# mit-acl/clipper

Hardware: AMD Instinct MI355X
Metric: affinity+solve ms and GEMV HBM GB/s, n=10k assoc, 95% outliers, 1/8 GPU (lower is better)
Workload: dtype f64 (M stored f32)

## Files before the change

### clipper_amd/build.py

```python
from __future__ import annotations

import os
import shutil
import subprocess
import sys
import sysconfig

HERE = os.path.dirname(os.path.abspath(__file__))
ROOT = os.path.dirname(HERE)
CSRC = os.path.join(HERE, "csrc")
LIBDIR = os.path.join(HERE, "lib")
HIP_LIB = os.path.join(LIBDIR, "libclipper_hip.so")
WAVE_CHECK_SRC = os.path.join(ROOT, "tests", "hip", "wave_check.hip")
WAVE_CHECK = os.path.join(ROOT, "tools", "_bin", "wave_check")

HIPCC = shutil.which("hipcc") or "/opt/rocm/bin/hipcc"
HIP_FLAGS = ["--offload-arch=gfx950", "-O3", "-std=c++17", "-ffp-contract=off", "-fPIC",
             "-shared", "-Wall", "-Wno-unused-value"]


def _newer(target: str, sources: list[str]) -> bool:
    if not os.path.exists(target):
        return False
    t = os.path.getmtime(target)
    return all(os.path.getmtime(s) <= t for s in sources if os.path.exists(s))


def _run(cmd: list[str]):
    print("+", " ".join(cmd), flush=True)
    subprocess.check_call(cmd)


def hip_sources() -> list[str]:
    return [os.path.join(dp, f) for top in (CSRC, os.path.join(ROOT, "include")) for dp, _, fs in os.walk(top)
            for f in fs if f.endswith((".hip", ".h", ".hpp"))]


def build_hip(force: bool = False) -> str:
    os.makedirs(LIBDIR, exist_ok=True)
    if force or not _newer(HIP_LIB, hip_sources()):
        _run([HIPCC, *HIP_FLAGS, "-o", HIP_LIB, os.path.join(CSRC, "clipper_hip.hip"), "-ldl"])
    return HIP_LIB


def pymodule_path() -> str:
    return os.path.join(LIBDIR, "clipperpy" + (sysconfig.get_config_var("EXT_SUFFIX") or ".so"))


def build_pymodule(force: bool = False) -> str | None:
    host = os.path.join(CSRC, "host")
    src = os.path.join(host, "py_clipper.cpp")
    if not os.path.exists(src):
        return None
    import pybind11
    out = pymodule_path()
    srcs = [src, os.path.join(host, "clipper.cpp"), os.path.join(host, "batch.cpp")] + [
        os.path.join(dp, f) for dp, _, fs in os.walk(os.path.join(ROOT, "include")) for f in fs]
    if force or not _newer(out, srcs + [HIP_LIB]):
        _run(["g++", "-O2", "-std=c++17", "-fPIC", "-shared", "-fvisibility=hidden", "-fopenmp",
              "-DCLIPPER_NO_EIGEN",
              "-I", os.path.join(ROOT, "include"), "-I", pybind11.get_include(),
              "-I", sysconfig.get_paths()["include"],
              src, os.path.join(host, "clipper.cpp"), os.path.join(host, "batch.cpp"),
              "-L", LIBDIR, "-lclipper_hip", "-Wl,-rpath,$ORIGIN", "-o", out])
    return out


def build_wave_check(force: bool = False) -> str:
    os.makedirs(os.path.dirname(WAVE_CHECK), exist_ok=True)
    if force or not _newer(WAVE_CHECK, hip_sources() + [WAVE_CHECK_SRC]):
        _run([HIPCC, *[f for f in HIP_FLAGS if f not in ("-shared", "-fPIC")], "-I", CSRC, "-o", WAVE_CHECK, WAVE_CHECK_SRC])
    return WAVE_CHECK


def build_all(force: bool = False):
    build_hip(force)
    build_pymodule(force)
    build_wave_check(force)


if __name__ == "__main__":
    build_all(force="--force" in sys.argv)
```

### clipper_amd/csrc/host_plan.hpp

```cpp
#pragma once

#include <algorithm>
#include <cmath>
#include <cstdint>
#include <cstdlib>
#include <vector>

namespace clipper_plan {

struct Work {
  int strip, slot, t0, t1;
  int q0, q1, pad0, pad1;
};

struct PassConsts {
  int nw;
  int so;
  int occ = 6;
  int per_strip = 12;
};

struct PassPlan {
  std::vector<Work> work;
  int nslots = 1;
// ... 237 lines not shown
        const size_t wv = ui * NWV + static_cast<size_t>(wave);
        out.wave_cg[wv] = static_cast<uint8_t>(cgl);
        int rem = (sub == nw[cgl] - 1) ? (1 << 30) : target, n = 0;
        while (rem > 0 && kcur < U.k1) {
          const int mq = static_cast<int>(lrow[kcur] & 255u);
          if (qcur >= mq) {
            ++kcur;
            qcur = 0;
            continue;
          }
          if (n == K.pmax) {
            if (sub == nw[cgl] - 1) return;
            break;
          }
          const int take = std::min(rem, mq - qcur);
          out.pieces[wv * PM + static_cast<size_t>(n++)] = static_cast<uint32_t>(kcur - U.k0) |
                                                           (static_cast<uint32_t>(qcur) << 8) |
                                                           (static_cast<uint32_t>(qcur + take) << 16);
          qcur += take;
          rem -= take;
        }
        out.npieces[wv] = static_cast<uint8_t>(n);
      }
    }
  }
  out.ok = true;
}


struct ViewUnit {
  int cg0, ncgs;
  int l0, l1;
  int pack;
  int pad1, pad2, pad3;
};

struct ViewResidentPlan {
  bool ok = false;
  uint32_t lds_slices = 0;
  uint64_t entries = 0;
  std::vector<ViewUnit> units;
  std::vector<uint8_t> npieces;
  std::vector<uint8_t> wave_cg;
  std::vector<uint32_t> pieces;
  std::vector<uint64_t> ent, byt;
  std::vector<int> stp, sorted_stp, T, nw;
};

inline void plan_view_resident(const uint32_t* L, int ncg, int nchunks, int esize, int target_units, int max_units,
                               uint32_t fixed_bytes, const ResidentConsts& K, ViewResidentPlan& out) {
  out.ok = false;
  out.units.clear();
  out.entries = 0;
  if (ncg < 1 || nchunks < 1 || nchunks > K.tmax || fixed_bytes + K.slice_pad + 8192 >= K.lds_max) return;
  const uint32_t cap = K.lds_max - fixed_bytes - K.slice_pad;
  out.lds_slices = K.lds_max - fixed_bytes;
  const uint32_t QBY = 4u * static_cast<uint32_t>(esize);
  std::vector<uint64_t>&ent = out.ent, &byt = out.byt;
  ent.assign(static_cast<size_t>(ncg), 0);
  byt.assign(static_cast<size_t>(ncg), 0);
  uint64_t total = 0;
  for (int cg = 0; cg < ncg; ++cg) {
    uint64_t e = 0, b = 0;
    for (int k = 0; k < nchunks; ++k) {
      const uint32_t lq = L[static_cast<size_t>(cg) * nchunks + k];
      e += lq >> 8;
      b += slice_bound(lq, QBY, K.so);
    }
    ent[static_cast<size_t>(cg)] = e;
    byt[static_cast<size_t>(cg)] = b;
    total += e;
  }
  out.entries = total;
  target_units = std::max(1, std::min(target_units, max_units));
  const double Te0 = std::max(256.0, static_cast<double>(total) / target_units);
  const int max_cgs = std::min(K.nwv, K.tmax / nchunks);
  if (max_cgs < 1) return;
  std::vector<int>&stp = out.stp, &sorted_stp = out.sorted_stp;
  stp.assign(static_cast<size_t>(ncg), 0);
  for (int c = 0; c < ncg; ++c) {
    int t = 0;
    for (int k = 0; k < nchunks; ++k) t += static_cast<int>(L[static_cast<size_t>(c) * nchunks + k] & 255u);
    stp[static_cast<size_t>(c)] = t;
  }
  sorted_stp = stp;
// ... 76 lines not shown
          best = cgl;
      ++nw[static_cast<size_t>(best)];
    }
    int wave = 0;
    for (int cgl = 0; cgl < U.ncgs; ++cgl) {
      const int nwc = nw[static_cast<size_t>(cgl)];
      const int target = std::max(1, (T[static_cast<size_t>(cgl)] + nwc - 1) / nwc);
      int kcur = 0, qcur = 0;
      for (int sub = 0; sub < nwc; ++sub, ++wave) {
        const size_t wv = ui * NWV + static_cast<size_t>(wave);
        out.wave_cg[wv] = static_cast<uint8_t>(cgl);
        int rem = (sub == nwc - 1) ? (1 << 30) : target, n = 0;
        while (rem > 0 && kcur < nsl) {
          const int mq = steps_of(cgl, kcur);
          if (qcur >= mq) {
            ++kcur;
            qcur = 0;
            continue;
          }
          if (n == K.pmax) {
            if (sub == nwc - 1) return;
            break;
          }
          const int take = std::min(rem, mq - qcur);
          out.pieces[wv * PM + static_cast<size_t>(n++)] = static_cast<uint32_t>(kcur) | (static_cast<uint32_t>(qcur) << 8) |
                                                           (static_cast<uint32_t>(qcur + take) << 16);
          qcur += take;
          rem -= take;
        }
        out.npieces[wv] = static_cast<uint8_t>(n);
      }
    }
  }
  out.ok = true;
}

}
```

### clipper_amd/csrc/host_rv_resident.hpp

```cpp
#pragma once

namespace {

void rvr_begin_solve(Ctx* h) {
  ViewResident& r = h->vres;
  r.launches_this_solve = 0;
  r.ev_n = 0;
  if (r.giveup_host) std::memset(r.giveup_host, 0, RVR_GIVEUP_SLOTS * 4 * sizeof(uint32_t));
  std::atomic_thread_fence(std::memory_order_seq_cst);
}

void rvr_end_solve(Ctx* h) {
  ViewResident& r = h->vres;
  if (r.cooldown > 0 && r.launches_this_solve == 0) --r.cooldown;
  if (r.launches_this_solve == 0 || !r.giveup_host) return;
  std::atomic_thread_fence(std::memory_order_acquire);
  int gave_up = 0;
  volatile const uint32_t* w = r.giveup_host;
  for (int k = 0; k < std::min(r.launches_this_solve, RVR_GIVEUP_SLOTS); ++k) {
    if (w[4 * k] != 0u) {
      ++gave_up;
    } else {
      h->rv_stats.resident_iterations += static_cast<int64_t>(w[4 * k + 1]);
      h->rv_stats.resident_us += static_cast<double>(static_cast<uint64_t>(w[4 * k + 2]) | (static_cast<uint64_t>(w[4 * k + 3]) << 32)) * 1e-2;
// ... 21 lines not shown
}

bool rvr_gate(const Ctx* h) { return h->rv_mode == 0 && csc_possible(h) && h->sh.size() == 1 && (h->V == 6 || h->V == 4); }
bool rvr_local_ok(const Ctx* h) {
  static const bool env_off = [] {
    const char* e = std::getenv("CLIPPER_HIP_VIEW_RESIDENT");
    return e && std::atoi(e) == 0;
  }();
  return !env_off && h->vres.cooldown == 0;
}
bool rvr_common(const Ctx* h) { return rvr_gate(h) && rvr_local_ok(h); }
bool rvr_enabled(const Ctx* h) { return rvr_common(h) && csc_single(h); }
bool rvr_replica_gate(const Ctx* h) { return rvr_gate(h) && h->multiproc && rect_fill_possible(h); }
bool rvr_replica_enabled(const Ctx* h) { return rvr_replica_gate(h) && rvr_local_ok(h); }

bool rvr_candidate(const Ctx* h, int64_t nrows) { return rvr_enabled(h) && nrows >= 1 && nrows <= RVR_MAXROWS; }

int rvr_plan(Ctx* h, Shard& s, bool replica = false) {
  ViewResident& r = h->vres;
  r.ready = false;
  r.on_replica = replica;
  if (!(replica ? rvr_replica_enabled(h) && s.rv.full_valid : rvr_enabled(h)) || !s.rv.valid) return 0;
  const RowView& v = s.rv;
  const SliceStore& vst = replica ? v.full : v.st;
  if (v.nrows < 1 || v.nrows > RVR_MAXROWS) return 0;
  static_assert(sizeof(clipper_plan::ViewUnit) == sizeof(RvrUnit), "the planner's unit is the kernel's");
  const clipper_plan::ResidentConsts K{RVR_NT, RVR_NWV, RVR_TMAX, RVR_PMAX, 2, RS_LDS_MAX,
                                       RVR_RED_BYTES, RVR_TAB_BYTES, RS_SLICE_PAD, SL_SO};
  static thread_local clipper_plan::ViewResidentPlan plan;
  if (r.target_units == 0) {
    const char* e = std::getenv("CLIPPER_HIP_VIEW_RESIDENT_WGS");
    r.target_units = e ? std::max(1, std::atoi(e)) : -1;
  }
  if (r.max_units_device < 0) {
    int per_cu = 0;
    hipError_t e = hipErrorUnknown;
    dispatch_vt(h, [&](auto tag) {
      using VT = decltype(tag);
      auto kern = (h->V == 6) ? k_solve_view_resident<VT, 6, false> : k_solve_view_resident<VT, 4, false>;
      if (raise_dynamic_lds(reinterpret_cast<const void*>(kern), s.device, static_cast<int>(RS_LDS_MAX)))
        e = hipOccupancyMaxActiveBlocksPerMultiprocessor(&per_cu, reinterpret_cast<const void*>(kern), RVR_NT, RS_LDS_MAX);
    });
    if (e != hipSuccess) (void)hipGetLastError();
    r.max_units_device = (e == hipSuccess) ? per_cu * h->cus : 0;
    if (rs_debug()) std::fprintf(stderr, "[view-resident] the device holds %d workgroups of the kernel at a time\n", r.max_units_device);
  }
  if (r.max_units_device < 16) return 0;
  const int max_units = std::min({RVR_MAXUNITS, h->cus - 8, r.max_units_device - 8});
  const int target = r.target_units > 0 ? r.target_units : std::max(8, (2 * h->cus) / 3);
  const uint32_t fixed = rvr_xt_bytes(h->V, static_cast<int>(v.nrows)) + RVR_RED_BYTES + RVR_TAB_BYTES;
  clipper_plan::plan_view_resident(h->csc_hLq, vst.s_ncg, vst.s_nchunks, static_cast<int>(h->esize()), target,
                                   max_units, fixed, K, plan);
  if (rs_debug())
    std::fprintf(stderr, "[view-resident] plan rows=%lld ncg=%d nchunks=%d entries=%llu -> units=%zu ok=%d\n",
                 static_cast<long long>(v.nrows), vst.s_ncg, vst.s_nchunks,
                 static_cast<unsigned long long>(plan.entries), plan.units.size(), plan.ok ? 1 : 0);
  if (!plan.ok) return 0;
  if (rs_debug() && std::atoi(std::getenv("CLIPPER_HIP_RESIDENT_DEBUG")) >= 2) {
    for (size_t ui = 0; ui < plan.units.size(); ++ui) {
      const clipper_plan::ViewUnit& U = plan.units[ui];
      uint64_t ent = 0;
      for (int c = 0; c < U.ncgs; ++c) ent += plan.ent[static_cast<size_t>(U.cg0 + c)];
      if (U.l1 - U.l0 < 64) ent = ent * static_cast<uint64_t>(U.l1 - U.l0) / 64;
      int wmax = 0, wsum = 0;
      for (int w = 0; w < RVR_NWV; ++w) {
        int st = 0;
        for (int j = 0; j < plan.npieces[ui * RVR_NWV + w]; ++j) {
          const uint32_t pc = plan.pieces[(ui * RVR_NWV + w) * RVR_PMAX + j];
          st += static_cast<int>((pc >> 16) & 255u) - static_cast<int>((pc >> 8) & 255u);
        }
        wmax = std::max(wmax, st);
        wsum += st;
      }
      std::fprintf(stderr, "[view-resident-unit] %zu cg0 %d ncgs %d lanes %d-%d pack %d entries %llu steps_max_wave %d steps_sum %d\n", ui, U.cg0, U.ncgs,
                   U.l0, U.l1, U.pack, static_cast<unsigned long long>(ent), wmax, wsum);
    }
  }
  HIPCHK(hipSetDevice(s.device));
  const size_t off_np = plan.units.size() * sizeof(RvrUnit);
  const size_t off_wc = off_np + static_cast<size_t>(round_up(static_cast<int64_t>(plan.npieces.size()), 16));
  const size_t off_pc = off_wc + static_cast<size_t>(round_up(static_cast<int64_t>(plan.wave_cg.size()), 16));
  const size_t bytes = off_pc + plan.pieces.size() * sizeof(uint32_t) + 64;
  if (bytes > r.host_plan.cap) HIPCHK(r.host_plan.alloc(bytes + 4096, hipHostMallocMapped | hipHostMallocCoherent));
  std::memcpy(r.host_plan, plan.units.data(), plan.units.size() * sizeof(RvrUnit));
  std::memcpy(r.host_plan + off_np, plan.npieces.data(), plan.npieces.size());
  std::memcpy(r.host_plan + off_wc, plan.wave_cg.data(), plan.wave_cg.size());
  {
    uint32_t* dst = reinterpret_cast<uint32_t*>(r.host_plan + off_pc);
    const uint32_t* src = plan.pieces.data();
    for (size_t wv = 0; wv < plan.npieces.size(); ++wv)
      for (int j = 0; j < plan.npieces[wv]; ++j) dst[wv * RVR_PMAX + j] = src[wv * RVR_PMAX + j];
  }
  std::atomic_thread_fence(std::memory_order_seq_cst);
  r.off_np = off_np;
  r.off_wc = off_wc;
  r.off_pc = off_pc;
  const size_t xb_bytes = static_cast<size_t>(rvr_xb_granules(6)) * sizeof(unsigned long long);
  if (!r.xb) {
    HIPCHK(r.xb.alloc(xb_bytes / sizeof(unsigned long long)));
    HIPCHK(hipMemsetAsync(r.xb, 0, xb_bytes, s.stream));
  }
  if (!r.ctl) {
    HIPCHK(r.ctl.alloc(RVR_GIVEUP_SLOTS * 16));
    HIPCHK(hipMemsetAsync(r.ctl, 0, RVR_GIVEUP_SLOTS * 64, s.stream));
  }
  if (!r.giveup_host) {
    HIPCHK(r.giveup_host.alloc(RVR_GIVEUP_SLOTS * 4, hipHostMallocMapped | hipHostMallocCoherent));
    std::memset(r.giveup_host, 0, RVR_GIVEUP_SLOTS * 4 * sizeof(uint32_t));
// ... 183 lines not shown
```

### clipper_amd/csrc/host_state.hpp

```cpp
#pragma once

namespace {

thread_local std::string g_err;

int fail(int code, const char* fmt, ...) {
  char buf[512];
  va_list ap;
  va_start(ap, fmt);
  vsnprintf(buf, sizeof(buf), fmt, ap);
  va_end(ap);
  g_err = buf;
  return code;
}

int guard_fail(int code, const char* what) noexcept {
  try {
    g_err = what;
  } catch (...) {
  }
  return code;
}
#define CLIPPER_HIP_GUARD_CATCH(on_nomem, on_other)                                                     \
  catch (const std::bad_alloc&) { on_nomem; }                                                            \
// ... 137 lines not shown

struct StagedInputs {
  const double* D1 = nullptr;
  const double* D2 = nullptr;
  const int32_t* A = nullptr;
};

struct Resident {
  bool ready = false;
  bool failed = false;
  int last_error = 0;
  int V = 0, E = 0, nunits = 0, maxslots = 0;
  uint32_t lds_slices = 0, lds_total = 0;
  PinnedBuf<uint8_t> host_plan;
  size_t off_np = 0, off_wc = 0, off_pc = 0;
  DevBuf<unsigned long long> xb;
  DevBuf<unsigned long long> ctl;
  unsigned long long epoch = 0;
  int V_forced = 0;
  bool xcd_off = false;
  int home = -1;
};

struct ViewResident {
  bool ready = false;
  int nunits = 0;
  uint32_t lds_slices = 0;
  PinnedBuf<uint8_t> host_plan;
  size_t off_np = 0, off_wc = 0, off_pc = 0;
  DevBuf<unsigned long long> xb;
  DevBuf<uint32_t> ctl;
  unsigned long long epoch = 0;
  int target_units = 0;
  PinnedBuf<uint32_t> giveup_host;
  Event ev[2 * 16];
  int ev_n = 0;
  uint64_t plan_entries = 0;
  int launches_this_solve = 0;
  int cooldown = 0, cooldown_next = 1;
  int max_units_device = -1;
  bool on_replica = false;
  DevBuf<uint8_t> backup;
};
constexpr int RVR_GIVEUP_SLOTS = 16;

constexpr int SUB_MAX_ENTRIES = 4;
constexpr int64_t SUB_MIN_M = 12000;
struct SubBufs {
  DevBuf<int32_t> cnt;
  DevBuf<uint8_t> flags;
  DevBuf<int32_t> colmap;
  DevBuf<int32_t> pos;
  DevBuf<uint32_t> blk;
  DevBuf<int32_t> nout_acc;
  PinnedBuf<SubRecord> rec;
};
struct SubProblem : SubBufs {
  struct clipper_hip_ctx* ctx = nullptr;
  struct clipper_hip_ctx* ctx_dense = nullptr;
  struct clipper_hip_ctx* use = nullptr;
  bool ready = false;
  bool active = false;
  int entries = 0;
  int launches_since_entry = 0;
  int64_t nS = 0;
  double ncol = 0.0;
// ... 118 lines not shown
```

### clipper_amd/csrc/k_rv_resident.hip.h

```cpp
#pragma once

#include <hip/hip_runtime.h>
#include <stdint.h>

#include "k_wave.hip.h"
#include "k_resident.hip.h"

namespace clipper_hip {

constexpr int RVR_NT = RS_NT;
constexpr int RVR_NWV = RS_NWV;
constexpr int RVR_TMAX = RS_TMAX;
constexpr int RVR_PMAX = RS_PMAX;
constexpr int RVR_MAXROWS = 2 * RVR_NT;
constexpr int RVR_MAXUNITS = 256;
constexpr int RVR_NRED = 40;

struct RvrUnit {
  int cg0, ncgs;
  int l0, l1;
  int pack;
  int pad1, pad2, pad3;
};

struct RvrArgs {
  SliceView R;
  const RvrUnit* units;
  int nunits;
  const uint32_t* pieces;
  const uint8_t* npieces;
  const uint8_t* wave_cg;
  const int32_t* viewpos;
  SolverState* st;
  SolveShared* shared;
  HostMirror* host;
  double* host_u;
  SolverParams prm;
  int64_t m, mp;
  double* pt;
  unsigned long long* xb;
  unsigned long long epoch0;
  uint32_t* ctl;
  uint32_t* giveup_host;
  uint32_t lds_slices;
  long long timeout_ticks;
  int max_exchanges;
  ViewPolicy rvp;
  int rv_rows;
  long long* stamps;
  const uint8_t* marks;
  uint8_t* kind;
  int64_t marks_n;
};
constexpr int RVR_FINE0 = 5120, RVR_FINE_TURNS = 96;
enum : int {
// ... 44 lines not shown
__device__ __forceinline__ void rvr_publish(unsigned long long* gq, unsigned long long tag, double x) {
  const unsigned long long bits = static_cast<unsigned long long>(__double_as_longlong(x));
  __hip_atomic_store(gq, tag | (bits >> 32), __ATOMIC_RELAXED, __HIP_MEMORY_SCOPE_AGENT);
  __hip_atomic_store(gq + 1, tag | (bits & 0xffffffffull), __ATOMIC_RELAXED, __HIP_MEMORY_SCOPE_AGENT);
}
__device__ __forceinline__ bool rvr_poll(const unsigned long long* gq, unsigned long long tag, double& x) {
  const unsigned long long g0 = rs_ld_granule(gq), g1 = rs_ld_granule(gq + 1);
  x = __longlong_as_double(static_cast<long long>((g0 << 32) | (g1 & 0xffffffffull)));
  return ((g0 ^ tag) >> 32) == 0 && ((g1 ^ tag) >> 32) == 0;
}

typedef uint32_t rvr_u4 __attribute__((ext_vector_type(4)));
__device__ __forceinline__ rvr_u4 rvr_ld16(const unsigned long long* gq) {
  rvr_u4 v;
  asm volatile("global_load_dwordx4 %0, %1, off sc1" : "=v"(v) : "v"(gq) : "memory");
  return v;
}
__device__ __forceinline__ void rvr_wait_loads() { asm volatile("s_waitcnt vmcnt(0)" ::: "memory"); }
__device__ __forceinline__ void rvr_tie(rvr_u4& v) { asm volatile("" : "+v"(v)); }
__device__ __forceinline__ bool rvr_take(const rvr_u4& v, uint32_t tag32, double& x) {
  x = __hiloint2double(static_cast<int>(v.x), static_cast<int>(v.z));
  return v.y == tag32 && v.w == tag32;
}
__device__ __forceinline__ int wave_isum_to_lane63(int v) {
  v += __builtin_amdgcn_update_dpp(0, v, 0xB1, 0xf, 0xf, false);
  v += __builtin_amdgcn_update_dpp(0, v, 0x4E, 0xf, 0xf, false);
  v += __builtin_amdgcn_update_dpp(0, v, 0x141, 0xf, 0xf, false);
  v += __builtin_amdgcn_update_dpp(0, v, 0x140, 0xf, 0xf, false);
  v += __builtin_amdgcn_update_dpp(0, v, 0x142, 0xa, 0xf, false);
  v += __builtin_amdgcn_update_dpp(0, v, 0x143, 0xc, 0xf, false);
  return v;
}

template <typename VT, int V, bool FINE>
__global__ __launch_bounds__(RVR_NT) void k_solve_view_resident(RvrArgs A) {
  extern __shared__ __attribute__((aligned(16))) uint8_t rvr_lds[];
  constexpr int NS = V + 1;
  constexpr int QB = 4 * static_cast<int>(sizeof(VT));
  typedef uint32_t u32x4 __attribute__((ext_vector_type(4)));
  static_assert(V >= 2 && V <= 6 && (V % 2) == 0, "window of the streaming solver on slices");
  const int tid = threadIdx.x, lane = tid & 63;
  const int wave = __builtin_amdgcn_readfirstlane(tid >> 6);
  const int64_t m = A.m, mp = A.mp;
  const int nrows = static_cast<int>(A.R.nrows);
  const SolverParams P = A.prm;
  const int unit = blockIdx.x;
  const bool two = nrows > RVR_NT;

  uint32_t off = 0;
  double* Xt = reinterpret_cast<double*>(rvr_lds + off);
  double* scr = Xt;
  off += rvr_xt_bytes(V, nrows);
  double* red = reinterpret_cast<double*>(rvr_lds + off);
  double* tot = red + RVR_NWV * RVR_NRED;
  double* nrmL = tot + 32;
  double* sxL = tot + 40;
  off += RVR_RED_BYTES;
  uint32_t* tab = reinterpret_cast<uint32_t*>(rvr_lds + off);
  uint32_t* words = tab + RVR_TMAX;
  uint32_t* sizes = words + 16;
  off += RVR_TAB_BYTES;
  uint8_t* sl = rvr_lds + off;

  const long long ts0 = wall_clock64();
  if (unit == 0 && tid == 0)
    __hip_atomic_store(reinterpret_cast<unsigned long long*>(A.ctl + 4), static_cast<unsigned long long>(ts0), __ATOMIC_RELAXED, __HIP_MEMORY_SCOPE_AGENT);
  const SolverState* st = A.st;
  const int e_done = A.shared->done, e_hold = st->hold, e_stage = st->stage, e_resume = st->resume;
  if (e_done || e_hold || e_stage != ST_PASS || (e_resume != 1 && e_resume != 2) || st->nout != 0 ||
      nrows > RVR_MAXROWS || nrows < 1 || P.maxiniters < 1)
    return;

  const RvrUnit U = A.units[unit];
  const unsigned long long wcg = *reinterpret_cast<const unsigned long long*>(A.wave_cg + static_cast<int64_t>(unit) * RVR_NWV);
  const int cgl = static_cast<int>((wcg >> (8 * wave)) & 255ull);
  const bool has_cg = cgl < U.ncgs && U.cg0 + cgl < A.R.ncg;
  const int G = U.pack > 1 ? U.pack : 1;
  const int Wd = U.l1 - U.l0;
  const int S = (A.R.nchunks + G - 1) / G;
  const int nslices = U.ncgs * S;
  const bool whole = U.l0 <= 0 && U.l1 >= 64;
  const bool packed = G > 1;
  const int lgrp = packed ? lane / Wd : 0;
  const int lsrc = packed ? U.l0 + (lane - lgrp * Wd) : lane;
  const bool in_lanes = packed ? true : (lane >= U.l0 && lane < U.l1);
  const gbytes_t rdata = (gbytes_t)A.R.data;
  const CLIPPER_GLOBAL uint64_t* rpre = (const CLIPPER_GLOBAL uint64_t*)A.R.Pre;
  auto src_of = [&](int t) -> gbytes_t {
    const int tc = t / S, tk = t - tc * S;
    return rdata + 16 * rpre[static_cast<int64_t>(U.cg0 + tc) * A.R.nchunks + tk];
  };
  auto src_chunk = [&](int k) -> gbytes_t {
    return rdata + 16 * rpre[static_cast<int64_t>(U.cg0) * A.R.nchunks + k];
  };
  if (nslices <= RVR_TMAX) {
    for (int t = wave; t < nslices; t += RVR_NWV) {
      uint32_t bytes = 0;
      if (packed) {
        const int k = t * G + lgrp;
        const bool have = k < A.R.nchunks;
        const gbytes_t sp = src_chunk(have ? k : 0);
        int mq = have ? static_cast<int>(reinterpret_cast<const CLIPPER_GLOBAL uint32_t*>(sp)[1]) : 0;
        const int tq = have ? static_cast<int>(sp[16 + lsrc]) : 0;
        mq = wave_max(mq);
        bytes = 16 + 64 + sl_so_bytes(mq) + sl_steps_bytes(tq, mq, QB);
        if (lane == 0) sizes[t] = bytes;
        continue;
      }
      const gbytes_t sp = src_of(t);
      const uint32_t nb = reinterpret_cast<const CLIPPER_GLOBAL uint32_t*>(sp)[2];
      bytes = nb;
      if (!whole) {
        const int maxq = __builtin_amdgcn_readfirstlane(static_cast<int>(reinterpret_cast<const CLIPPER_GLOBAL uint32_t*>(sp)[1]));
        const int tq = in_lanes ? static_cast<int>(sp[16 + lane]) : 0;
        bytes = 16 + 64 + sl_so_bytes(maxq) + sl_steps_bytes(tq, maxq, QB);
      }
      if (lane == 0) sizes[t] = bytes;
    }
  }
  __syncthreads();
  if (wave == 0) {
    const uint32_t bytes_t = (lane < nslices && nslices <= RVR_TMAX) ? sizes[lane] : 0u;
    const uint32_t inc = wave_scan_incl(bytes_t);
    tab[lane] = inc - bytes_t;
    if (lane == 63) words[0] = inc;
  }
  __syncthreads();
  const uint32_t total = words[0];
  const bool bad_plan = total + RS_SLICE_PAD > A.lds_slices || nslices > RVR_TMAX || U.ncgs > RVR_NWV;
  if (__syncthreads_or(bad_plan ? 1 : 0)) {
    if (tid == 0) {
      __hip_atomic_store(A.ctl, static_cast<uint32_t>(RVR_ERR_LDS), __ATOMIC_RELAXED, __HIP_MEMORY_SCOPE_AGENT);
      if (A.giveup_host) __hip_atomic_store(A.giveup_host, static_cast<uint32_t>(RVR_ERR_LDS), __ATOMIC_RELAXED, __HIP_MEMORY_SCOPE_SYSTEM);
    }
    return;
  }
  for (int t = wave; t < nslices; t += RVR_NWV) {
    const uint32_t o = tab[t];
    if (packed) {
      const int k = t * G + lgrp;
      const bool have = k < A.R.nchunks;
      const gbytes_t src = src_chunk(have ? k : 0);
      const int mq_own = have ? static_cast<int>(reinterpret_cast<const CLIPPER_GLOBAL uint32_t*>(src)[1]) : 0;
      const int tot_dst = have ? static_cast<int>(src[16 + lsrc]) : 0;
      const int maxq = __builtin_amdgcn_readfirstlane(wave_max(mq_own));
      uint8_t* dp = sl + o;
      if (lane < 4) reinterpret_cast<uint32_t*>(dp)[lane] = (lane == 1) ? static_cast<uint32_t>(maxq) : 0u;
      dp[16 + lane] = static_cast<uint8_t>(tot_dst);
      for (int b = lane * 4; b < sl_so_bytes(maxq); b += 256) *reinterpret_cast<uint32_t*>(dp + 16 + 64 + b) = 0u;
      uint8_t* dfb = dp + 16 + 64 + sl_so_bytes(maxq);
      gbytes_t sfb = src + 16 + 64 + sl_so_bytes(mq_own);
      int tgs[8];
#pragma unroll
      for (int g = 0; g < 8; ++g) {
        const int kg = t * G + g;
        tgs[g] = (g < G && kg < A.R.nchunks) ? static_cast<int>(src_chunk(kg)[16 + lane]) : 0;
      }
      for (int q = 0; q < maxq; ++q) {
        uint64_t ms_own = 0;
#pragma unroll
        for (int g = 0; g < 8; ++g) {
          const uint64_t mg = __ballot(q < tgs[g]);
          if (g == lgrp) ms_own = mg;
        }
        const bool ad = q < tot_dst;
        const uint64_t md = __ballot(ad);
        const int cd = __builtin_amdgcn_readfirstlane(__popcll(md));
        const int cs = __popcll(ms_own);
        if (ad) {
          const uint32_t rs_ = static_cast<uint32_t>(__popcll(ms_own & ((1ull << lsrc) - 1ull)));
          const uint32_t rd_ = sl_lane_rank(md);
          SliceQuad<VT> vq;
          vq.load(sfb + rs_ * QB);
          const uint32_t rq = *reinterpret_cast<const CLIPPER_GLOBAL uint32_t*>(sfb + cs * QB + rs_ * 4);
          vq.store(dfb + rd_ * QB);
          *reinterpret_cast<uint32_t*>(dfb + cd * QB + rd_ * 4) = rq;
        }
        sfb += cs * QB + ((cs * 4 + 15) & ~15);
        dfb += cd * QB + ((cd * 4 + 15) & ~15);
      }
      continue;
    }
    const gbytes_t src = src_of(t);
    if (whole) {
      const uint32_t nb = reinterpret_cast<const CLIPPER_GLOBAL uint32_t*>(src)[2];
      for (uint32_t b = lane * 16; b < nb; b += 64 * 16)
        *reinterpret_cast<u32x4*>(sl + o + b) = *reinterpret_cast<const CLIPPER_GLOBAL u32x4*>(src + b);
    } else {
      const int maxq = __builtin_amdgcn_readfirstlane(static_cast<int>(reinterpret_cast<const CLIPPER_GLOBAL uint32_t*>(src)[1]));
      const int tot_src = static_cast<int>(src[16 + lane]);
      const int tot_dst = in_lanes ? tot_src : 0;
      uint8_t* dp = sl + o;
      if (lane < 4) reinterpret_cast<uint32_t*>(dp)[lane] = (lane == 1) ? static_cast<uint32_t>(maxq) : 0u;
      dp[16 + lane] = static_cast<uint8_t>(tot_dst);
      for (int b = lane * 4; b < sl_so_bytes(maxq); b += 256) *reinterpret_cast<uint32_t*>(dp + 16 + 64 + b) = 0u;
      gbytes_t sfb = src + 16 + 64 + sl_so_bytes(maxq);
      uint8_t* dfb = dp + 16 + 64 + sl_so_bytes(maxq);
      for (int q = 0; q < maxq; ++q) {
        const bool as = q < tot_src, ad = q < tot_dst;
        const uint64_t ms = __ballot(as), md = __ballot(ad);
        const int cs = __builtin_amdgcn_readfirstlane(__popcll(ms)), cd = __builtin_amdgcn_readfirstlane(__popcll(md));
        if (ad) {
          const uint32_t rs_ = sl_lane_rank(ms), rd_ = sl_lane_rank(md);
          SliceQuad<VT> vq;
          vq.load(sfb + rs_ * QB);
          const uint32_t rq = *reinterpret_cast<const CLIPPER_GLOBAL uint32_t*>(sfb + cs * QB + rs_ * 4);
          vq.store(dfb + rd_ * QB);
          *reinterpret_cast<uint32_t*>(dfb + cd * QB + rd_ * 4) = rq;
        }
        sfb += cs * QB + ((cs * 4 + 15) & ~15);
        dfb += cd * QB + ((cd * 4 + 15) & ~15);
      }
    }
  }
  const uint32_t* toff = tab + (has_cg ? cgl * S : 0);
  const int np = has_cg ? A.npieces[unit * RVR_NWV + wave] : 0;
  const uint32_t pc = (lane < RVR_PMAX) ? A.pieces[(static_cast<int64_t>(unit) * RVR_NWV + wave) * RVR_PMAX + lane] : 0u;

  double d = st->d, F = st->F, alpha = st->alpha, s = st->s;
  int i_ = st->i, j_ = st->j, k_ = st->k;
  const int e_ubp = st->ubp, e_ubv = st->ubv;
  int64_t n_passes = st->n_passes, n_trials = st->n_trials, n_iters = st->n_iters, n_view_passes = st->n_view_passes;
  int nlive = st->nlive, nout = 0;
  const int rv_builds = st->rv_builds, rv_last = st->rv_last, rv_backoff = st->rv_backoff;
  const int n_redo = st->n_redo;

  const double* Ue = A.pt + ((static_cast<int64_t>(e_ubp) * V + e_ubv) * 2 + 0) * mp;
  const double* Ge = A.pt + ((static_cast<int64_t>(e_ubp) * V + e_ubv) * 2 + 1) * mp;
  double UR[2], GR[2], aR[2] = {0.0, 0.0}, bR[2] = {0.0, 0.0};
  bool rok[2];
#pragma unroll
  for (int e = 0; e < 2; ++e) {
    const int r = tid + e * RVR_NT;
    rok[e] = r < nrows;
    const int64_t i = rok[e] ? A.R.rowmap[r] : 0;
    UR[e] = rok[e] ? Ue[i] : 0.0;
    GR[e] = rok[e] ? Ge[i] : 0.0;
  }
  const int64_t col = static_cast<int64_t>(U.cg0 + wave) * 64 + (packed ? U.l0 + lane : lane);
  const bool cown = wave < U.ncgs && (packed ? lane < Wd : in_lanes) && col < m;
  const int rpos = cown ? A.viewpos[col] : -1;
  double u_c = cown ? Ue[col] : 0.0, g_c = cown ? Ge[col] : 0.0, a_c = 0.0, b_c = 0.0;
  __syncthreads();

  unsigned long long epoch = A.epoch0;
  int exchanges = 0;
  int stamp_row = 0;
  const long long ts1 = A.stamps ? wall_clock64() : 0;
  auto stamp_end = [&]() {
    if (A.stamps && unit == 0 && tid == 0) {
// ... 125 lines not shown
          HostMirror* hm = A.host;
          __hip_atomic_store(&hm->nlive, nlive, __ATOMIC_RELAXED, __HIP_MEMORY_SCOPE_SYSTEM);
          __hip_atomic_store(&hm->nout, nout, __ATOMIC_RELAXED, __HIP_MEMORY_SCOPE_SYSTEM);
          __hip_atomic_store(&hm->n_view_passes, n_view_passes, __ATOMIC_RELAXED, __HIP_MEMORY_SCOPE_SYSTEM);
          __hip_atomic_store(&hm->iters, n_iters, __ATOMIC_RELEASE, __HIP_MEMORY_SCOPE_SYSTEM);
        }
      }
      stamp_end();
      return;
    }

    fstamp_value(RVR_F_KIND, kind);
    double y[NS];
#pragma unroll
    for (int v = 0; v < NS; ++v) y[v] = 0.0;
    if (kind != K_BUILD) {
#pragma unroll
      for (int e = 0; e < 2; ++e) {
        const int r = tid + e * RVR_NT;
        if (r < nrows) {
          double al = alpha;
#pragma unroll
          for (int l = 0; l < V; ++l) {
            double t = cl_project(UR[e], al, GR[e]);
            if (kind == K_PAIR) t = (l == 0) ? UR[e] : 0.0;
            Xt[r * V + l] = t;
            al = al * P.beta;
          }
        }
      }
      __syncthreads();
      fstamp(RVR_F_XT);
      double acc[NS];
      rs_wave_pass<VT, V>(sl, toff, pc, np, 0, Xt, (kind == K_TRIAL) ? d : 0.0, acc, G, lgrp * SL_SUB);
      if constexpr (FINE) {
        if (A.stamps && unit == 0 && lane == 0 && trow < RVR_FINE_TURNS)
          A.stamps[RVR_FINE0 + trow * 32 + RVR_F_WAVE + wave] = wall_clock64() + (acc[0] > 1e300 ? 1 : 0);
      }
      if (wave < V) {
        double z = 0.0, t1 = 0.0;
        if (kind == K_TRIAL) {
          for (int r = lane; r < nrows; r += 64) {
            const double c = Xt[r * V + wave];
            z += c * c;
            t1 += c;
          }
          z = wave_sum_to_lane63(z);
          t1 = wave_sum_to_lane63(t1);
        }
        if (lane == 63) {
          const double nl = cl_norm(z, kind == K_TRIAL);
          nrmL[wave] = nl;
          sxL[wave] = (kind == K_TRIAL) ? t1 / nl : 0.0;
        }
      }
      __syncthreads();
      fstamp(RVR_F_NORMS);
      if (packed) {
        for (int o = Wd; o < 64; o <<= 1) {
#pragma unroll
          for (int v = 0; v < NS; ++v) acc[v] += __shfl_xor(acc[v], o);
        }
      }
#pragma unroll
      for (int v = 0; v < NS; ++v) scr[(wave * NS + v) * 64 + lane] = acc[v];
      __syncthreads();
      if (wave < U.ncgs) {
// ... 398 lines not shown
```

Before: 1.262.

## Add flat per-wave LDS slice layout for view-resident solver walk

When a unit's work fits in LDS, the view-resident kernel now decodes the compressed slices once at staging into a flat, fixed-stride per-wave layout with pre-expanded row indices. The per-iteration pass then runs a simple double-buffered loop over that layout instead of the compact walk with its ballot/popcount rank bookkeeping. The flat layout uses more LDS per unit, so units that do not fit fall back to the compact path. An environment variable can force the compact walk, and a walk-check test binary is added to the build.

```diff
diff --git a/clipper_amd/build.py b/clipper_amd/build.py
--- a/clipper_amd/build.py
+++ b/clipper_amd/build.py
@@ -13,6 +13,8 @@
 HIP_LIB = os.path.join(LIBDIR, "libclipper_hip.so")
 WAVE_CHECK_SRC = os.path.join(ROOT, "tests", "hip", "wave_check.hip")
 WAVE_CHECK = os.path.join(ROOT, "tools", "_bin", "wave_check")
+RVR_WALK_CHECK_SRC = os.path.join(ROOT, "tests", "hip", "rvr_walk_check.hip")
+RVR_WALK_CHECK = os.path.join(ROOT, "tools", "_bin", "rvr_walk_check")
 
 HIPCC = shutil.which("hipcc") or "/opt/rocm/bin/hipcc"
 HIP_FLAGS = ["--offload-arch=gfx950", "-O3", "-std=c++17", "-ffp-contract=off", "-fPIC",
@@ -73,10 +75,18 @@
     return WAVE_CHECK
 
 
+def build_rvr_walk_check(force: bool = False) -> str:
+    os.makedirs(os.path.dirname(RVR_WALK_CHECK), exist_ok=True)
+    if force or not _newer(RVR_WALK_CHECK, hip_sources() + [RVR_WALK_CHECK_SRC]):
+        _run([HIPCC, *[f for f in HIP_FLAGS if f not in ("-shared", "-fPIC")], "-I", CSRC, "-o", RVR_WALK_CHECK, RVR_WALK_CHECK_SRC])
+    return RVR_WALK_CHECK
+
+
 def build_all(force: bool = False):
     build_hip(force)
     build_pymodule(force)
     build_wave_check(force)
+    build_rvr_walk_check(force)
 
 
 if __name__ == "__main__":
diff --git a/clipper_amd/csrc/host_plan.hpp b/clipper_amd/csrc/host_plan.hpp
--- a/clipper_amd/csrc/host_plan.hpp
+++ b/clipper_amd/csrc/host_plan.hpp
@@ -293,8 +293,23 @@
   int cg0, ncgs;
   int l0, l1;
   int pack;
-  int pad1, pad2, pad3;
-};
+  int flat;
+  int pad2, pad3;
+};
+
+inline uint32_t view_flat_stride(int esize) { return 64u * (4u * static_cast<uint32_t>(esize) + 8u); }
+inline void view_flat_regions(const uint32_t* pieces , const uint8_t* npieces , int nwv,
+                              int pmax, int esize, uint64_t* off ) {
+  off[0] = 0;
+  for (int w = 0; w < nwv; ++w) {
+    uint64_t st = 0;
+    for (int j = 0; j < npieces[w]; ++j) {
+      const uint32_t pc = pieces[static_cast<size_t>(w) * pmax + j];
+      st += ((pc >> 16) & 255u) - ((pc >> 8) & 255u);
+    }
+    off[w + 1] = off[w] + st * view_flat_stride(esize);
+  }
+}
 
 struct ViewResidentPlan {
   bool ok = false;
@@ -304,14 +319,18 @@
   std::vector<uint8_t> npieces;
   std::vector<uint8_t> wave_cg;
   std::vector<uint32_t> pieces;
+  std::vector<uint64_t> flat_bytes;
+  int nflat = 0;
   std::vector<uint64_t> ent, byt;
   std::vector<int> stp, sorted_stp, T, nw;
 };
 
 inline void plan_view_resident(const uint32_t* L, int ncg, int nchunks, int esize, int target_units, int max_units,
-                               uint32_t fixed_bytes, const ResidentConsts& K, ViewResidentPlan& out) {
+                               uint32_t fixed_bytes, const ResidentConsts& K, ViewResidentPlan& out, bool allow_flat = true) {
   out.ok = false;
   out.units.clear();
+  out.flat_bytes.clear();
+  out.nflat = 0;
   out.entries = 0;
   if (ncg < 1 || nchunks < 1 || nchunks > K.tmax || fixed_bytes + K.slice_pad + 8192 >= K.lds_max) return;
   const uint32_t cap = K.lds_max - fixed_bytes - K.slice_pad;
@@ -454,6 +473,14 @@
       }
     }
   }
+  out.flat_bytes.assign(units.size(), 0);
+  std::vector<uint64_t> off(NWV + 1);
+  for (size_t ui = 0; ui < units.size(); ++ui) {
+    view_flat_regions(out.pieces.data() + ui * NWV * PM, out.npieces.data() + ui * NWV, K.nwv, K.pmax, esize, off.data());
+    out.flat_bytes[ui] = off[NWV];
+    units[ui].flat = (allow_flat && off[NWV] <= cap) ? 1 : 0;
+    out.nflat += units[ui].flat;
+  }
   out.ok = true;
 }
 
diff --git a/clipper_amd/csrc/host_rv_resident.hpp b/clipper_amd/csrc/host_rv_resident.hpp
--- a/clipper_amd/csrc/host_rv_resident.hpp
+++ b/clipper_amd/csrc/host_rv_resident.hpp
@@ -77,6 +77,10 @@
     const char* e = std::getenv("CLIPPER_HIP_VIEW_RESIDENT_WGS");
     r.target_units = e ? std::max(1, std::atoi(e)) : -1;
   }
+  if (r.walk_compact < 0) {
+    const char* e = std::getenv("CLIPPER_HIP_VIEW_RESIDENT_WALK");
+    r.walk_compact = (e && std::strcmp(e, "compact") == 0) ? 1 : 0;
+  }
   if (r.max_units_device < 0) {
     int per_cu = 0;
     hipError_t e = hipErrorUnknown;
@@ -95,11 +99,11 @@
   const int target = r.target_units > 0 ? r.target_units : std::max(8, (2 * h->cus) / 3);
   const uint32_t fixed = rvr_xt_bytes(h->V, static_cast<int>(v.nrows)) + RVR_RED_BYTES + RVR_TAB_BYTES;
   clipper_plan::plan_view_resident(h->csc_hLq, vst.s_ncg, vst.s_nchunks, static_cast<int>(h->esize()), target,
-                                   max_units, fixed, K, plan);
+                                   max_units, fixed, K, plan, r.walk_compact == 0);
   if (rs_debug())
-    std::fprintf(stderr, "[view-resident] plan rows=%lld ncg=%d nchunks=%d entries=%llu -> units=%zu ok=%d\n",
+    std::fprintf(stderr, "[view-resident] plan rows=%lld ncg=%d nchunks=%d entries=%llu -> units=%zu (%d flat) ok=%d\n",
                  static_cast<long long>(v.nrows), vst.s_ncg, vst.s_nchunks,
-                 static_cast<unsigned long long>(plan.entries), plan.units.size(), plan.ok ? 1 : 0);
+                 static_cast<unsigned long long>(plan.entries), plan.units.size(), plan.ok ? plan.nflat : 0, plan.ok ? 1 : 0);
   if (!plan.ok) return 0;
   if (rs_debug() && std::atoi(std::getenv("CLIPPER_HIP_RESIDENT_DEBUG")) >= 2) {
     for (size_t ui = 0; ui < plan.units.size(); ++ui) {
@@ -117,8 +121,9 @@
         wmax = std::max(wmax, st);
         wsum += st;
       }
-      std::fprintf(stderr, "[view-resident-unit] %zu cg0 %d ncgs %d lanes %d-%d pack %d entries %llu steps_max_wave %d steps_sum %d\n", ui, U.cg0, U.ncgs,
-                   U.l0, U.l1, U.pack, static_cast<unsigned long long>(ent), wmax, wsum);
+      std::fprintf(stderr, "[view-resident-unit] %zu cg0 %d ncgs %d lanes %d-%d pack %d entries %llu steps_max_wave %d steps_sum %d walk %s flat_bytes %llu\n", ui, U.cg0, U.ncgs,
+                   U.l0, U.l1, U.pack, static_cast<unsigned long long>(ent), wmax, wsum, U.flat ? "flat" : "compact",
+                   static_cast<unsigned long long>(plan.flat_bytes[ui]));
     }
   }
   HIPCHK(hipSetDevice(s.device));
diff --git a/clipper_amd/csrc/host_state.hpp b/clipper_amd/csrc/host_state.hpp
--- a/clipper_amd/csrc/host_state.hpp
+++ b/clipper_amd/csrc/host_state.hpp
@@ -193,6 +193,7 @@
   DevBuf<uint32_t> ctl;
   unsigned long long epoch = 0;
   int target_units = 0;
+  int walk_compact = -1;
   PinnedBuf<uint32_t> giveup_host;
   Event ev[2 * 16];
   int ev_n = 0;
diff --git a/clipper_amd/csrc/k_rv_resident.hip.h b/clipper_amd/csrc/k_rv_resident.hip.h
--- a/clipper_amd/csrc/k_rv_resident.hip.h
+++ b/clipper_amd/csrc/k_rv_resident.hip.h
@@ -20,7 +20,8 @@
   int cg0, ncgs;
   int l0, l1;
   int pack;
-  int pad1, pad2, pad3;
+  int flat;
+  int pad2, pad3;
 };
 
 struct RvrArgs {
@@ -131,73 +132,234 @@
   return v;
 }
 
-template <typename VT, int V, bool FINE>
-__global__ __launch_bounds__(RVR_NT) void k_solve_view_resident(RvrArgs A) {
-  extern __shared__ __attribute__((aligned(16))) uint8_t rvr_lds[];
-  constexpr int NS = V + 1;
+constexpr uint32_t RVR_FLAT_NONE = 0xffffffffu;
+__host__ __device__ constexpr uint32_t rvr_flat_stride(int esize) { return 64u * (4u * static_cast<uint32_t>(esize) + 8u); }
+
+template <typename VT, int V>
+__device__ __forceinline__ void rvr_flat_pass(const uint8_t* fb, int ns, const double* Xt, double d, double (&acc)[V + 1]) {
+  constexpr int QB = 4 * static_cast<int>(sizeof(VT));
+  constexpr int FS = static_cast<int>(rvr_flat_stride(sizeof(VT)));
+  const int lane = threadIdx.x & 63;
+#pragma unroll
+  for (int v = 0; v <= V; ++v) acc[v] = 0.0;
+  if (ns <= 0) return;
+  const uint8_t* pv = fb + lane * QB;
+  const uint8_t* pr = fb + 64 * QB + lane * 8;
+  auto issue = [&](int s, SliceQuad<VT>& vq, uint2& rq) {
+    const int sc = min(s, ns - 1);
+    vq.load(pv + sc * FS);
+    rq = *reinterpret_cast<const uint2*>(pr + sc * FS);
+  };
+  auto mult = [&](int s, const SliceQuad<VT>& vq, const uint2& rq) {
+    if (s < ns && rq.x != RVR_FLAT_NONE) {
+#pragma unroll
+      for (int e = 0; e < 4; ++e) {
+        const VT mf = vq.v[e];
+        const double mm = static_cast<double>(mf);
+        const double ii = mf != VT(0) ? 1.0 : 0.0;
+        const uint32_t row = ((e < 2 ? rq.x : rq.y) >> (16 * (e & 1))) & 0xffffu;
+        const double* xr = Xt + row * V;
+        double xv[V];
+#pragma unroll
+        for (int v = 0; v < V; v += 2) {
+          const double2 t2 = *reinterpret_cast<const double2*>(xr + v);
+          xv[v] = t2.x;
+          xv[v + 1] = t2.y;
+        }
+        acc[0] = fma(mm, xv[0], acc[0]);
+        acc[V] = fma(ii, xv[0], acc[V]);
+        const double w = fma(d, ii, mm);
+#pragma unroll
+        for (int v = 1; v < V; ++v) acc[v] = fma(w, xv[v], acc[v]);
+      }
+    }
+  };
+  SliceQuad<VT> cur, nxt, nx2, nx3;
+  uint2 rcur, rnxt, r2, r3;
+  issue(0, cur, rcur);
+  issue(1, nxt, rnxt);
+  for (int s = 0; s < ns; s += 2) {
+    issue(s + 2, nx2, r2);
+    issue(s + 3, nx3, r3);
+    mult(s, cur, rcur);
+    mult(s + 1, nxt, rnxt);
+    cur = nx2;
+    rcur = r2;
+    nxt = nx3;
+    rnxt = r3;
+  }
+}
+
+template <typename VT>
+struct RvrPieceHead {
+  gbytes_t src;
+  int k;
+  int mq_own;
+  int tot_dst;
+  int tgs[8];
+};
+template <typename VT>
+__device__ __forceinline__ RvrPieceHead<VT> rvr_flat_head(gbytes_t rdata, unsigned long long dirv , int nchunks,
+                                                          uint32_t piece, int G, int lgrp, int lsrc, bool in_lanes) {
+  const int lane = threadIdx.x & 63;
+  const int kl = static_cast<int>(piece & 255u);
+  RvrPieceHead<VT> H;
+  H.k = kl * G + lgrp;
+  const bool have = H.k < nchunks;
+  H.src = rdata + 16 * __shfl(dirv, have ? H.k : 0);
+  H.mq_own = have ? static_cast<int>(reinterpret_cast<const CLIPPER_GLOBAL uint32_t*>(H.src)[1]) : 0;
+  H.tot_dst = (have && in_lanes) ? static_cast<int>(H.src[16 + lsrc]) : 0;
+#pragma unroll
+  for (int g = 0; g < 8; ++g) {
+    const int kg = kl * G + g;
+    const bool hg = g < G && kg < nchunks;
+    const gbytes_t sg = rdata + 16 * __shfl(dirv, hg ? kg : 0);
+    H.tgs[g] = hg ? static_cast<int>(sg[16 + lane]) : 0;
+  }
+  return H;
+}
+template <typename VT>
+__device__ __forceinline__ int rvr_flat_decode(const RvrPieceHead<VT>& H, uint32_t piece, int lgrp, int lsrc, uint8_t* fb, int s0) {
+  constexpr int QB = 4 * static_cast<int>(sizeof(VT));
+  constexpr int FS = static_cast<int>(rvr_flat_stride(sizeof(VT)));
+  const int lane = threadIdx.x & 63;
+  const int q0 = static_cast<int>((piece >> 8) & 255u);
+  const int mq_own = H.mq_own, tot_dst = H.tot_dst;
+  const int maxq = __builtin_amdgcn_readfirstlane(wave_max(mq_own));
+  const int q1 = min(static_cast<int>((piece >> 16) & 255u), maxq);
+  const uint64_t below = (1ull << lsrc) - 1ull;
+  const uint32_t row0 = static_cast<uint32_t>(H.k * SL_SUB) * 0x10001u;
+  auto active_own = [&](int q) -> uint64_t {
+    uint64_t ms_own = 0;
+#pragma unroll
+    for (int g = 0; g < 8; ++g) {
+      const uint64_t mg = __ballot(q < H.tgs[g]);
+      if (g == lgrp) ms_own = mg;
+    }
+    return ms_own;
+  };
+  gbytes_t sfb = H.src + 16 + 64 + sl_so_bytes(mq_own);
+  for (int q = 0; q < q0; ++q) {
+    const int cs = __popcll(active_own(q));
+    sfb += cs * QB + ((cs * 4 + 15) & ~15);
+  }
+  for (int qb = q0; qb < q1; qb += 4) {
+    SliceQuad<VT> vq[4];
+    uint32_t rq[4];
+    bool ad[4];
+#pragma unroll
+    for (int b = 0; b < 4; ++b) {
+      const int q = qb + b;
+      const uint64_t ms_own = (q < q1) ? active_own(q) : 0ull;
+      ad[b] = q < q1 && q < tot_dst;
+      const int cs = __popcll(ms_own);
+      const uint32_t rs_ = ad[b] ? static_cast<uint32_t>(__popcll(ms_own & below)) : 0u;
+      vq[b].load(sfb + rs_ * QB);
+      rq[b] = *reinterpret_cast<const CLIPPER_GLOBAL uint32_t*>(sfb + cs * QB + rs_ * 4);
+      sfb += cs * QB + ((cs * 4 + 15) & ~15);
+    }
+#pragma unroll
+    for (int b = 0; b < 4; ++b) {
+      if (qb + b < q1) {
+        uint8_t* dp = fb + (s0 + qb + b - q0) * FS;
+        uint2 rw = make_uint2(RVR_FLAT_NONE, RVR_FLAT_NONE);
+        if (ad[b]) {
+          vq[b].store(dp + lane * QB);
+          rw.x = row0 + ((rq[b] & 0xffu) | ((rq[b] & 0xff00u) << 8));
+          rw.y = row0 + (((rq[b] >> 16) & 0xffu) | ((rq[b] >> 8) & 0xff0000u));
+        }
+        *reinterpret_cast<uint2*>(dp + 64 * QB + lane * 8) = rw;
+      }
+    }
+  }
+  return q1 > q0 ? q1 - q0 : 0;
+}
+
+struct RvrLanes {
+  int G;
+  int Wd;
+  int S;
+  bool whole, packed;
+  int lgrp;
+  int lsrc;
+  bool in_lanes;
+};
+__device__ __forceinline__ RvrLanes rvr_lanes(const RvrUnit& U, int nchunks, int lane) {
+  RvrLanes L;
+  L.G = U.pack > 1 ? U.pack : 1;
+  L.Wd = U.l1 - U.l0;
+  L.S = (nchunks + L.G - 1) / L.G;
+  L.whole = U.l0 <= 0 && U.l1 >= 64;
+  L.packed = L.G > 1;
+  L.lgrp = L.packed ? lane / L.Wd : 0;
+  L.lsrc = L.packed ? U.l0 + (lane - L.lgrp * L.Wd) : lane;
+  L.in_lanes = L.packed ? true : (lane >= U.l0 && lane < U.l1);
+  return L;
+}
+
+template <typename VT>
+__device__ __forceinline__ bool rvr_flat_stage(gbytes_t rdata, const CLIPPER_GLOBAL uint64_t* rpre, int nchunks, const RvrUnit& U,
+                                               const RvrLanes& L, int cgl, int np, uint32_t pc, uint32_t* words ,
+                                               uint8_t* sl, uint32_t lds_slices, const uint8_t*& fl_base, int& fl_ns) {
+  const int lane = threadIdx.x & 63;
+  const int wave = __builtin_amdgcn_readfirstlane(threadIdx.x >> 6);
+  constexpr uint32_t FS = rvr_flat_stride(sizeof(VT));
+  const CLIPPER_GLOBAL uint64_t* dir = rpre + static_cast<int64_t>(U.cg0 + cgl) * nchunks;
+  const unsigned long long dirv = lane < nchunks ? dir[lane] : 0ull;
+  uint32_t piece = np > 0 ? static_cast<uint32_t>(__builtin_amdgcn_readlane(static_cast<int>(pc), 0)) : 0u;
+  RvrPieceHead<VT> cur = rvr_flat_head<VT>(rdata, dirv, nchunks, piece, L.G, L.lgrp, L.lsrc, L.in_lanes);
+  int stp = (lane < np) ? static_cast<int>((pc >> 16) & 255u) - static_cast<int>((pc >> 8) & 255u) : 0;
+  stp = wave_isum_to_lane63(stp < 0 ? 0 : stp);
+  if (lane == 63) words[4 + wave] = static_cast<uint32_t>(stp);
+  __syncthreads();
+  uint32_t before = 0, steps_all = 0;
+#pragma unroll
+  for (int w = 0; w < RVR_NWV; ++w) {
+    const uint32_t sw = words[4 + w];
+    before += (w < wave) ? sw : 0u;
+    steps_all += sw;
+  }
+  before = __builtin_amdgcn_readfirstlane(before);
+  const bool bad_plan = static_cast<uint64_t>(steps_all) * FS + RS_SLICE_PAD > lds_slices || U.ncgs > RVR_NWV;
+  if (__syncthreads_or(bad_plan ? 1 : 0)) return false;
+  uint8_t* fb = sl + before * FS;
+  int s_ = 0;
+  for (int j = 0; j < np; ++j) {
+    const uint32_t pnext = static_cast<uint32_t>(__builtin_amdgcn_readlane(static_cast<int>(pc), j + 1 < np ? j + 1 : j));
+    const RvrPieceHead<VT> nxt = rvr_flat_head<VT>(rdata, dirv, nchunks, pnext, L.G, L.lgrp, L.lsrc, L.in_lanes);
+    s_ += rvr_flat_decode<VT>(cur, piece, L.lgrp, L.lsrc, fb, s_);
+    cur = nxt;
+    piece = pnext;
+  }
+  fl_base = fb;
+  fl_ns = __builtin_amdgcn_readfirstlane(s_);
+  return true;
+}
+
+template <typename VT>
+__device__ __forceinline__ bool rvr_compact_stage(gbytes_t rdata, const CLIPPER_GLOBAL uint64_t* rpre, int nchunks, const RvrUnit& U,
+                                                  const RvrLanes& L, uint32_t* tab, uint32_t* words, uint32_t* sizes, uint8_t* sl,
+                                                  uint32_t lds_slices) {
   constexpr int QB = 4 * static_cast<int>(sizeof(VT));
   typedef uint32_t u32x4 __attribute__((ext_vector_type(4)));
-  static_assert(V >= 2 && V <= 6 && (V % 2) == 0, "window of the streaming solver on slices");
-  const int tid = threadIdx.x, lane = tid & 63;
-  const int wave = __builtin_amdgcn_readfirstlane(tid >> 6);
-  const int64_t m = A.m, mp = A.mp;
-  const int nrows = static_cast<int>(A.R.nrows);
-  const SolverParams P = A.prm;
-  const int unit = blockIdx.x;
-  const bool two = nrows > RVR_NT;
-
-  uint32_t off = 0;
-  double* Xt = reinterpret_cast<double*>(rvr_lds + off);
-  double* scr = Xt;
-  off += rvr_xt_bytes(V, nrows);
-  double* red = reinterpret_cast<double*>(rvr_lds + off);
-  double* tot = red + RVR_NWV * RVR_NRED;
-  double* nrmL = tot + 32;
-  double* sxL = tot + 40;
-  off += RVR_RED_BYTES;
-  uint32_t* tab = reinterpret_cast<uint32_t*>(rvr_lds + off);
-  uint32_t* words = tab + RVR_TMAX;
-  uint32_t* sizes = words + 16;
-  off += RVR_TAB_BYTES;
-  uint8_t* sl = rvr_lds + off;
-
-  const long long ts0 = wall_clock64();
-  if (unit == 0 && tid == 0)
-    __hip_atomic_store(reinterpret_cast<unsigned long long*>(A.ctl + 4), static_cast<unsigned long long>(ts0), __ATOMIC_RELAXED, __HIP_MEMORY_SCOPE_AGENT);
-  const SolverState* st = A.st;
-  const int e_done = A.shared->done, e_hold = st->hold, e_stage = st->stage, e_resume = st->resume;
-  if (e_done || e_hold || e_stage != ST_PASS || (e_resume != 1 && e_resume != 2) || st->nout != 0 ||
-      nrows > RVR_MAXROWS || nrows < 1 || P.maxiniters < 1)
-    return;
-
-  const RvrUnit U = A.units[unit];
-  const unsigned long long wcg = *reinterpret_cast<const unsigned long long*>(A.wave_cg + static_cast<int64_t>(unit) * RVR_NWV);
-  const int cgl = static_cast<int>((wcg >> (8 * wave)) & 255ull);
-  const bool has_cg = cgl < U.ncgs && U.cg0 + cgl < A.R.ncg;
-  const int G = U.pack > 1 ? U.pack : 1;
-  const int Wd = U.l1 - U.l0;
-  const int S = (A.R.nchunks + G - 1) / G;
+  const int lane = threadIdx.x & 63;
+  const int wave = __builtin_amdgcn_readfirstlane(threadIdx.x >> 6);
+  const int G = L.G, S = L.S, lgrp = L.lgrp, lsrc = L.lsrc;
+  const bool whole = L.whole, packed = L.packed, in_lanes = L.in_lanes;
   const int nslices = U.ncgs * S;
-  const bool whole = U.l0 <= 0 && U.l1 >= 64;
-  const bool packed = G > 1;
-  const int lgrp = packed ? lane / Wd : 0;
-  const int lsrc = packed ? U.l0 + (lane - lgrp * Wd) : lane;
-  const bool in_lanes = packed ? true : (lane >= U.l0 && lane < U.l1);
-  const gbytes_t rdata = (gbytes_t)A.R.data;
-  const CLIPPER_GLOBAL uint64_t* rpre = (const CLIPPER_GLOBAL uint64_t*)A.R.Pre;
   auto src_of = [&](int t) -> gbytes_t {
     const int tc = t / S, tk = t - tc * S;
-    return rdata + 16 * rpre[static_cast<int64_t>(U.cg0 + tc) * A.R.nchunks + tk];
+    return rdata + 16 * rpre[static_cast<int64_t>(U.cg0 + tc) * nchunks + tk];
   };
   auto src_chunk = [&](int k) -> gbytes_t {
-    return rdata + 16 * rpre[static_cast<int64_t>(U.cg0) * A.R.nchunks + k];
+    return rdata + 16 * rpre[static_cast<int64_t>(U.cg0) * nchunks + k];
   };
   if (nslices <= RVR_TMAX) {
     for (int t = wave; t < nslices; t += RVR_NWV) {
       uint32_t bytes = 0;
       if (packed) {
         const int k = t * G + lgrp;
-        const bool have = k < A.R.nchunks;
+        const bool have = k < nchunks;
         const gbytes_t sp = src_chunk(have ? k : 0);
         int mq = have ? static_cast<int>(reinterpret_cast<const CLIPPER_GLOBAL uint32_t*>(sp)[1]) : 0;
         const int tq = have ? static_cast<int>(sp[16 + lsrc]) : 0;
@@ -226,19 +388,13 @@
   }
   __syncthreads();
   const uint32_t total = words[0];
-  const bool bad_plan = total + RS_SLICE_PAD > A.lds_slices || nslices > RVR_TMAX || U.ncgs > RVR_NWV;
-  if (__syncthreads_or(bad_plan ? 1 : 0)) {
-    if (tid == 0) {
-      __hip_atomic_store(A.ctl, static_cast<uint32_t>(RVR_ERR_LDS), __ATOMIC_RELAXED, __HIP_MEMORY_SCOPE_AGENT);
-      if (A.giveup_host) __hip_atomic_store(A.giveup_host, static_cast<uint32_t>(RVR_ERR_LDS), __ATOMIC_RELAXED, __HIP_MEMORY_SCOPE_SYSTEM);
-    }
-    return;
-  }
+  const bool bad_plan = total + RS_SLICE_PAD > lds_slices || nslices > RVR_TMAX || U.ncgs > RVR_NWV;
+  if (__syncthreads_or(bad_plan ? 1 : 0)) return false;
   for (int t = wave; t < nslices; t += RVR_NWV) {
     const uint32_t o = tab[t];
     if (packed) {
       const int k = t * G + lgrp;
-      const bool have = k < A.R.nchunks;
+      const bool have = k < nchunks;
       const gbytes_t src = src_chunk(have ? k : 0);
       const int mq_own = have ? static_cast<int>(reinterpret_cast<const CLIPPER_GLOBAL uint32_t*>(src)[1]) : 0;
       const int tot_dst = have ? static_cast<int>(src[16 + lsrc]) : 0;
@@ -253,7 +409,7 @@
 #pragma unroll
       for (int g = 0; g < 8; ++g) {
         const int kg = t * G + g;
-        tgs[g] = (g < G && kg < A.R.nchunks) ? static_cast<int>(src_chunk(kg)[16 + lane]) : 0;
+        tgs[g] = (g < G && kg < nchunks) ? static_cast<int>(src_chunk(kg)[16 + lane]) : 0;
       }
       for (int q = 0; q < maxq; ++q) {
         uint64_t ms_own = 0;
@@ -312,9 +468,70 @@
       }
     }
   }
+  return true;
+}
+
+template <typename VT, int V, bool FINE>
+__global__ __launch_bounds__(RVR_NT) void k_solve_view_resident(RvrArgs A) {
+  extern __shared__ __attribute__((aligned(16))) uint8_t rvr_lds[];
+  constexpr int NS = V + 1;
+  static_assert(V >= 2 && V <= 6 && (V % 2) == 0, "window of the streaming solver on slices");
+  const int tid = threadIdx.x, lane = tid & 63;
+  const int wave = __builtin_amdgcn_readfirstlane(tid >> 6);
+  const int64_t m = A.m, mp = A.mp;
+  const int nrows = static_cast<int>(A.R.nrows);
+  const SolverParams P = A.prm;
+  const int unit = blockIdx.x;
+  const bool two = nrows > RVR_NT;
+
+  uint32_t off = 0;
+  double* Xt = reinterpret_cast<double*>(rvr_lds + off);
+  double* scr = Xt;
+  off += rvr_xt_bytes(V, nrows);
+  double* red = reinterpret_cast<double*>(rvr_lds + off);
+  double* tot = red + RVR_NWV * RVR_NRED;
+  double* nrmL = tot + 32;
+  double* sxL = tot + 40;
+  off += RVR_RED_BYTES;
+  uint32_t* tab = reinterpret_cast<uint32_t*>(rvr_lds + off);
+  uint32_t* words = tab + RVR_TMAX;
+  uint32_t* sizes = words + 16;
+  off += RVR_TAB_BYTES;
+  uint8_t* sl = rvr_lds + off;
+
+  const long long ts0 = wall_clock64();
+  if (unit == 0 && tid == 0)
+    __hip_atomic_store(reinterpret_cast<unsigned long long*>(A.ctl + 4), static_cast<unsigned long long>(ts0), __ATOMIC_RELAXED, __HIP_MEMORY_SCOPE_AGENT);
+  const SolverState* st = A.st;
+  const int e_done = A.shared->done, e_hold = st->hold, e_stage = st->stage, e_resume = st->resume;
+  if (e_done || e_hold || e_stage != ST_PASS || (e_resume != 1 && e_resume != 2) || st->nout != 0 ||
+      nrows > RVR_MAXROWS || nrows < 1 || P.maxiniters < 1)
+    return;
+
+  const RvrUnit U = A.units[unit];
+  const unsigned long long wcg = *reinterpret_cast<const unsigned long long*>(A.wave_cg + static_cast<int64_t>(unit) * RVR_NWV);
+  const int cgl = static_cast<int>((wcg >> (8 * wave)) & 255ull);
+  const bool has_cg = cgl < U.ncgs && U.cg0 + cgl < A.R.ncg;
+  const RvrLanes Ln = rvr_lanes(U, A.R.nchunks, lane);
+  const int G = Ln.G, Wd = Ln.Wd, S = Ln.S, lgrp = Ln.lgrp;
+  const bool packed = Ln.packed, in_lanes = Ln.in_lanes;
+  const gbytes_t rdata = (gbytes_t)A.R.data;
+  const CLIPPER_GLOBAL uint64_t* rpre = (const CLIPPER_GLOBAL uint64_t*)A.R.Pre;
   const uint32_t* toff = tab + (has_cg ? cgl * S : 0);
   const int np = has_cg ? A.npieces[unit * RVR_NWV + wave] : 0;
   const uint32_t pc = (lane < RVR_PMAX) ? A.pieces[(static_cast<int64_t>(unit) * RVR_NWV + wave) * RVR_PMAX + lane] : 0u;
+  const bool flat = U.flat != 0;
+  const uint8_t* fl_base = sl;
+  int fl_ns = 0;
+  const bool staged = flat ? rvr_flat_stage<VT>(rdata, rpre, A.R.nchunks, U, Ln, has_cg ? cgl : 0, np, pc, words, sl, A.lds_slices, fl_base, fl_ns)
+                           : rvr_compact_stage<VT>(rdata, rpre, A.R.nchunks, U, Ln, tab, words, sizes, sl, A.lds_slices);
+  if (!staged) {
+    if (tid == 0) {
+      __hip_atomic_store(A.ctl, static_cast<uint32_t>(RVR_ERR_LDS), __ATOMIC_RELAXED, __HIP_MEMORY_SCOPE_AGENT);
+      if (A.giveup_host) __hip_atomic_store(A.giveup_host, static_cast<uint32_t>(RVR_ERR_LDS), __ATOMIC_RELAXED, __HIP_MEMORY_SCOPE_SYSTEM);
+    }
+    return;
+  }
 
   double d = st->d, F = st->F, alpha = st->alpha, s = st->s;
   int i_ = st->i, j_ = st->j, k_ = st->k;
@@ -506,7 +723,8 @@
       __syncthreads();
       fstamp(RVR_F_XT);
       double acc[NS];
-      rs_wave_pass<VT, V>(sl, toff, pc, np, 0, Xt, (kind == K_TRIAL) ? d : 0.0, acc, G, lgrp * SL_SUB);
+      if (flat) rvr_flat_pass<VT, V>(fl_base, fl_ns, Xt, (kind == K_TRIAL) ? d : 0.0, acc);
+      else rs_wave_pass<VT, V>(sl, toff, pc, np, 0, Xt, (kind == K_TRIAL) ? d : 0.0, acc, G, lgrp * SL_SUB);
       if constexpr (FINE) {
         if (A.stamps && unit == 0 && lane == 0 && trow < RVR_FINE_TURNS)
           A.stamps[RVR_FINE0 + trow * 32 + RVR_F_WAVE + wave] = wall_clock64() + (acc[0] > 1e300 ? 1 : 0);
```

Result: no change. 1.241 (median of 3 runs) (-1.6%).
